# ZihanLiao/pytorch-kaldi-resnet

Measured on AMD Instinct MI355X. Metric: utterances/sec (300-frame x 80 fbank, bs256/GPU), ResNet-34 + AAM-softmax training step, higher is better.
Workload: dtype f32 (operands as 2 fp16 terms of value x 2^k, 3 cross products, f32 accumulate); 1 GPU; BASELINE configs[1]: ResNet-34 + AAM-softmax (m 0.2, s 30), 1211 speakers, 300-frame x 80 fbank, per-GPU batch 256, fwd+CE+bwd+SGD(0.9, wd 5e-4); global_batch=256, frames=300, feat_dim=80, parallelism=dp1, launch=hipGraph replay (1 graph), mfma=f16x3

## Files before the change

pytorch-kaldi-resnet_amd/csrc/conv3x3_c32_stream.hip:

```cpp
#include "spk_common.h"

struct Conv3x3C32Args {
    const float* in;
    const float* wpk;
    const unsigned* w_amax;
    float* out;
    const float* in_scale;
    const float* in_shift;
    float* stats;
    const unsigned* in_amax;
    unsigned* out_amax;
    int B, H, W, tiles_x, tiles_y, ntiles, flags;
};

#define C32_TH 8
#define C32_TW 16
#define C32_HW 18
#define C32_HP (10 * 18)
#define C32_PIX 144
#define C32_ROW 2816
#define C32_WBYTES (9 * 2 * 2 * 1024)
#ifndef C32_KD
#define C32_KD 2
#endif
#ifndef C32_DEPTH
#define C32_DEPTH 2
#endif

#ifdef C32_STAMPS
static __device__ unsigned long long g_c32_stamps[1024][8];
#define C32_T(i) do { const unsigned long long now_ = __builtin_amdgcn_s_memtime(); ph[i] += now_ - last; last = now_; } while (0)
#else
#define C32_T(i) do { } while (0)
#endif

#ifndef C32_XCD_BAND
#define C32_XCD_BAND 1
#endif
template <int VAR>
__global__ __launch_bounds__(256, 2) void conv3x3_c32_stream_kernel(Conv3x3C32Args a) {
    extern __shared__ __attribute__((aligned(16))) unsigned char lds3[];
    unsigned char* wl = lds3;
    unsigned char* hl = lds3 + C32_WBYTES;
    const int tid = threadIdx.x, lane = tid & 63;
    const int wave = __builtin_amdgcn_readfirstlane(tid >> 6);
    const int r = lane & 31, h = lane >> 5;
    constexpr bool AFF = VAR != 0;
    const float sig = spk_sigma_from_amax_bits(*a.in_amax);
    const float inv_sig = 1.f / sig, inv_wsig = 1.f / spk_sigma_from_amax_bits(*a.w_amax);
    const int H = a.H, W = a.W;

    for (int i = tid; i < C32_WBYTES / 16; i += 256) *(f32x4*)(wl + i * 16) = *(const f32x4*)(a.wpk + i * 4);

    const int q = tid & 7, prow = tid >> 3;
    int hy[6], hx[6];
    unsigned goff[6], loff[6];
#pragma unroll
    for (int u = 0; u < 6; ++u) {
        const int p = prow + 32 * u;
        const int pc = p < C32_HP ? p : C32_HP - 1;
        hy[u] = pc / C32_HW;
        hx[u] = pc - hy[u] * C32_HW;
        goff[u] = (unsigned)((hy[u] * W + hx[u]) * 32 + q * 4);
        loff[u] = (unsigned)(hy[u] * C32_ROW + hx[u] * C32_PIX + (q >> 2) * 64 + (q & 3) * 8);
    }
    const bool item5 = prow + 32 * 5 < C32_HP;
    f32x4 sc = {1.f, 1.f, 1.f, 1.f}, sh = {0.f, 0.f, 0.f, 0.f};
    if constexpr (AFF) {
        sc = *(const f32x4*)(a.in_scale + q * 4);
        sh = *(const f32x4*)(a.in_shift + q * 4);
    }

    f32x4 va[6], vb[6], vc[6];
    unsigned okma = 0, okmb = 0, okmc = 0;
    auto tile_origin = [&](int tile, int& b, int& y0, int& x0) {
        const int tx = tile % a.tiles_x;
        const int t2 = tile / a.tiles_x;
        const int ty = t2 % a.tiles_y;
        b = t2 / a.tiles_y;
        y0 = ty * C32_TH;
        x0 = tx * C32_TW;
    };
    auto issue = [&](int tile, f32x4* v, unsigned& okm) {
        int b, y0, x0;
        tile_origin(tile, b, y0, x0);
        const bool edge = y0 == 0 || y0 + C32_TH >= H || x0 == 0 || x0 + C32_TW >= W;
        const int base = ((b * H + y0 - 1) * W + x0 - 1) * 32;
        const int safe = ((b * H + y0) * W + x0) * 32 + q * 4;
        okm = 0x3f;
        if (!edge) {
#pragma unroll
            for (int u = 0; u < 6; ++u) v[u] = *(const f32x4*)(a.in + (unsigned)(base + (int)goff[u]));
        } else {
            okm = 0;
#pragma unroll
            for (int u = 0; u < 6; ++u) {
                const int iy = y0 - 1 + hy[u], ix = x0 - 1 + hx[u];
                const bool ok = iy >= 0 && iy < H && ix >= 0 && ix < W;
                okm |= (unsigned)ok << u;
                v[u] = *(const f32x4*)(a.in + (unsigned)(ok ? base + (int)goff[u] : safe));
            }
        }
    };

    double s_sum = 0.0, s_sq = 0.0;
    float out_mx = 0.f;
    const unsigned char* rd = hl + (2 * wave + (r >> 4)) * C32_ROW + (r & 15) * C32_PIX + h * 16;
    const unsigned char* wb = wl + lane * 16;

    const int G = (int)gridDim.x;
#ifdef C32_STAMPS
    unsigned long long ph[8] = {0, 0, 0, 0, 0, 0, 0, 0}, last = __builtin_amdgcn_s_memtime();
    const unsigned long long born = last;
#endif
    auto step = [&](int tile, f32x4* v, unsigned& okm) {
        int b, y0, x0;
        tile_origin(tile, b, y0, x0);
        C32_T(0);
        __syncthreads();
        C32_T(1);
#pragma unroll
        for (int u = 0; u < 6; ++u) {
#ifdef C32_ABL_NOSTAGE
            break;
#endif
            if (u == 5 && !item5) break;
            f32x4 w = v[u];
            if constexpr (AFF) {
                w = w * sc + sh;
                w[0] = fmaxf(w[0], 0.f);
                w[1] = fmaxf(w[1], 0.f);
                w[2] = fmaxf(w[2], 0.f);
                w[3] = fmaxf(w[3], 0.f);
            }
            if (!((okm >> u) & 1u)) w = (f32x4){0.f, 0.f, 0.f, 0.f};
            uint2 t0, t1;
            split2h(w, sig, t0, t1);
            *(uint2*)(hl + loff[u]) = t0;
            *(uint2*)(hl + loff[u] + 32) = t1;
        }
        C32_T(2);
        __syncthreads();
        C32_T(3);
#ifndef C32_ABL_NOLOAD
        if (tile + C32_DEPTH * G < a.ntiles) issue(tile + C32_DEPTH * G, v, okm);
#endif
        C32_T(4);

        f32x16 acc;
#pragma unroll
        for (int e = 0; e < 16; ++e) acc[e] = 0.f;
#ifdef C32_ABL_HALFK
        constexpr int NG = 1;
#else
        constexpr int NG = 2;
#endif
        constexpr int NS = NG * 9;
        f32x4 fr[C32_KD + 1][4];
        auto frag = [&](int s2, f32x4* f) {
            const int g = s2 / 9, t = s2 % 9;
            const int toff = (t / 3) * C32_ROW + (t % 3) * C32_PIX;
            f[0] = *(const f32x4*)(rd + toff + g * 64);
            f[1] = *(const f32x4*)(rd + toff + g * 64 + 32);
            f[2] = *(const f32x4*)(wb + ((t * 2 + g) * 2 + 0) * 1024);
            f[3] = *(const f32x4*)(wb + ((t * 2 + g) * 2 + 1) * 1024);
        };
#pragma unroll
        for (int s2 = 0; s2 < C32_KD; ++s2) frag(s2, fr[s2]);
#pragma unroll
        for (int s2 = 0; s2 < NS; ++s2) {
            if (s2 + C32_KD < NS) frag(s2 + C32_KD, fr[(s2 + C32_KD) % (C32_KD + 1)]);
            __builtin_amdgcn_sched_barrier(0);
            const f32x4* f = fr[s2 % (C32_KD + 1)];
            acc = __builtin_amdgcn_mfma_f32_32x32x16_f16(__builtin_bit_cast(f16x8, f[0]), __builtin_bit_cast(f16x8, f[3]), acc, 0, 0, 0);
            acc = __builtin_amdgcn_mfma_f32_32x32x16_f16(__builtin_bit_cast(f16x8, f[1]), __builtin_bit_cast(f16x8, f[2]), acc, 0, 0, 0);
            acc = __builtin_amdgcn_mfma_f32_32x32x16_f16(__builtin_bit_cast(f16x8, f[0]), __builtin_bit_cast(f16x8, f[2]), acc, 0, 0, 0);
            __builtin_amdgcn_sched_barrier(0);
        }

        C32_T(5);
        const bool ragged = y0 + C32_TH > H || x0 + C32_TW > W;
        float ts = 0.f, tq = 0.f, tile_mx = 0.f;
        float* ob = a.out + (size_t)((b * H + y0 + 2 * wave) * W + x0) * 32 + r;
#pragma unroll
        for (int e = 0; e < 16; ++e) {
            const int row = e >> 3, lx = (e & 3) + 8 * ((e >> 2) & 1) + 4 * h;
            if (ragged && (y0 + 2 * wave + row >= H || x0 + lx >= W)) continue;
            const float val = acc[e] * inv_sig * inv_wsig;
#ifndef C32_ABL_NOSTORE
            __builtin_nontemporal_store(val, ob + (row * W + lx) * 32);
#endif
            tile_mx = fmaxf(tile_mx, fabsf(val));
            ts += val;
            tq = __builtin_fmaf(val, val, tq);
        }
        if (__builtin_amdgcn_ballot_w64(!(tile_mx < __builtin_inff())) != 0) {
            tile_mx = 0.f;
#pragma unroll
            for (int e = 0; e < 16; ++e) {
                const int row = e >> 3, lx = (e & 3) + 8 * ((e >> 2) & 1) + 4 * h;
                if (ragged && (y0 + 2 * wave + row >= H || x0 + lx >= W)) continue;
                tile_mx = fmaxf(tile_mx, spk_finite_abs(acc[e] * inv_sig * inv_wsig));
            }
        }
        out_mx = fmaxf(out_mx, tile_mx);
        s_sum += (double)ts;
        s_sq += (double)tq;
        C32_T(6);
    };
    const int vblk = (C32_XCD_BAND && (G & 7) == 0) ? ((int)blockIdx.x & 7) * (G >> 3) + ((int)blockIdx.x >> 3) : (int)blockIdx.x;
    int tile = vblk;
    if (tile < a.ntiles) issue(tile, va, okma);
    if (tile + G < a.ntiles) issue(tile + G, vb, okmb);
    if (C32_DEPTH > 2 && tile + 2 * G < a.ntiles) issue(tile + 2 * G, vc, okmc);
    for (; tile < a.ntiles; tile += C32_DEPTH * G) {
        step(tile, va, okma);
        if (tile + G < a.ntiles) step(tile + G, vb, okmb);
        if (C32_DEPTH > 2 && tile + 2 * G < a.ntiles) step(tile + 2 * G, vc, okmc);
    }

#ifdef C32_STAMPS
    if (tid == 0 && blockIdx.x < 1024) {
        for (int i = 0; i < 7; ++i) g_c32_stamps[blockIdx.x][i] = ph[i];
        g_c32_stamps[blockIdx.x][7] = __builtin_amdgcn_s_memtime() - born;
    }
#endif
    if (a.out_amax) spk_wave_amax_commit(out_mx, a.out_amax);
    if (a.flags & SPK_EPI_STATS) {
        s_sum += __shfl_xor(s_sum, 32, 64);
        s_sq += __shfl_xor(s_sq, 32, 64);
        if (h == 0) {
            float* dst = a.stats + ((size_t)(vblk * 4 + wave) * 32 + r) * 2;
            dst[0] = (float)s_sum;
            dst[1] = (float)s_sq;
        }
    }
}

extern "C" int spk_conv3x3_c32_stream(const float* in, const float* wpk, float* out, const float* in_scale, const float* in_shift,
                                      float* stats , int B, int H, int W, int flags, const unsigned* in_amax,
                                      unsigned* out_amax, int nblocks, void* stream) {
    SPK_REQUIRE(in && wpk && out && in_amax, "spk_conv3x3_c32_stream: null pointer (in, wpk, out and the in_amax slot are required)");
    SPK_REQUIRE(B > 0 && H > 0 && W > 0 && (long long)B * H * W * 32 < 2147483647LL - 65536, "spk_conv3x3_c32_stream: %d x %d x %d pixels exceed 32-bit element offsets", B, H, W);
    SPK_REQUIRE((flags & ~(SPK_IN_AFFINE_RELU | SPK_EPI_STATS)) == 0, "spk_conv3x3_c32_stream: unsupported flags 0x%x", flags);
    SPK_REQUIRE(!(flags & SPK_IN_AFFINE_RELU) || (in_scale && in_shift), "spk_conv3x3_c32_stream: IN_AFFINE_RELU needs scale / shift");
    SPK_REQUIRE(!(flags & SPK_EPI_STATS) || stats, "spk_conv3x3_c32_stream: EPI_STATS needs a stats buffer");
    Conv3x3C32Args a;
    a.in = in; a.w_amax = (const unsigned*)wpk; a.wpk = wpk + 4; a.out = out; a.in_scale = in_scale; a.in_shift = in_shift;
    a.stats = stats; a.in_amax = in_amax; a.out_amax = out_amax; a.B = B; a.H = H; a.W = W; a.flags = flags;
    a.tiles_x = spk_ceil_div(W, C32_TW); a.tiles_y = spk_ceil_div(H, C32_TH);
    a.ntiles = B * a.tiles_y * a.tiles_x;
    SPK_REQUIRE(nblocks >= 1 && nblocks <= a.ntiles, "spk_conv3x3_c32_stream: nblocks=%d for %d tiles", nblocks, a.ntiles);
    const size_t lds_bytes = C32_WBYTES + 10 * C32_ROW;
    hipStream_t st = (hipStream_t)stream;
    if (flags & SPK_IN_AFFINE_RELU) hipLaunchKernelGGL(conv3x3_c32_stream_kernel<1>, dim3(nblocks), dim3(256), lds_bytes, st, a);
    else hipLaunchKernelGGL(conv3x3_c32_stream_kernel<0>, dim3(nblocks), dim3(256), lds_bytes, st, a);
    SPK_LAUNCH_CHECK("spk_conv3x3_c32_stream");
    return 0;
}

#ifdef C32_STAMPS
extern "C" int spk_debug_stamps_c32(unsigned long long* out, int nblocks) {
    if (nblocks < 0) {
        static unsigned long long zeros[1024][8];
        return (int)hipMemcpyToSymbol(HIP_SYMBOL(g_c32_stamps), zeros, sizeof(zeros));
    }
    return (int)hipMemcpyFromSymbol(out, HIP_SYMBOL(g_c32_stamps), sizeof(unsigned long long) * 8 * (size_t)nblocks);
}
#endif
```

Measured before the change: 5620 utt/s.

## Add optional 16x16x32 MFMA path and magic-number tile index division

Adds a compile-time C32_M16 variant of the 3x3 conv with 32 channels. It uses 16x16x32 f16 MFMAs over a 2x2 accumulator grid, with a new padded LDS layout for the halo and weights, per-lane stores of two output channels, and per-channel stats reduction. It also replaces the integer divide and modulo in tile_origin with multiply-high by precomputed reciprocals plus a correction step. The MFMA path is off by default (C32_M16=0), so only the cheaper tile index math runs by default.

New measurement: 5612 utt/s. About the same (-0.1%).

```diff
diff --git a/pytorch-kaldi-resnet_amd/csrc/conv3x3_c32_stream.hip b/pytorch-kaldi-resnet_amd/csrc/conv3x3_c32_stream.hip
--- a/pytorch-kaldi-resnet_amd/csrc/conv3x3_c32_stream.hip
+++ b/pytorch-kaldi-resnet_amd/csrc/conv3x3_c32_stream.hip
@@ -11,6 +11,7 @@
     const unsigned* in_amax;
     unsigned* out_amax;
     int B, H, W, tiles_x, tiles_y, ntiles, flags;
+    unsigned tiles_x_magic, tiles_y_magic;
 };
 
 #define C32_TH 8
@@ -20,8 +21,19 @@
 #define C32_PIX 144
 #define C32_ROW 2816
 #define C32_WBYTES (9 * 2 * 2 * 1024)
+#ifndef C32_M16
+#define C32_M16 0
+#endif
+#define C32M_PIX 160
+#define C32M_ROW (C32_HW * C32M_PIX)
+#define C32M_WROW 80
+#define C32M_WBYTES (9 * 2 * 32 * C32M_WROW)
 #ifndef C32_KD
+#if C32_M16
+#define C32_KD 1
+#else
 #define C32_KD 2
+#endif
 #endif
 #ifndef C32_DEPTH
 #define C32_DEPTH 2
@@ -40,17 +52,30 @@
 template <int VAR>
 __global__ __launch_bounds__(256, 2) void conv3x3_c32_stream_kernel(Conv3x3C32Args a) {
     extern __shared__ __attribute__((aligned(16))) unsigned char lds3[];
+#if C32_M16
+    unsigned char* wl = lds3;
+    unsigned char* hl = lds3 + C32M_WBYTES;
+#else
     unsigned char* wl = lds3;
     unsigned char* hl = lds3 + C32_WBYTES;
+#endif
     const int tid = threadIdx.x, lane = tid & 63;
     const int wave = __builtin_amdgcn_readfirstlane(tid >> 6);
     const int r = lane & 31, h = lane >> 5;
+    const int c16 = lane & 15, kq = lane >> 4;
     constexpr bool AFF = VAR != 0;
     const float sig = spk_sigma_from_amax_bits(*a.in_amax);
     const float inv_sig = 1.f / sig, inv_wsig = 1.f / spk_sigma_from_amax_bits(*a.w_amax);
     const int H = a.H, W = a.W;
 
+#if C32_M16
+    for (int i = tid; i < C32_WBYTES / 16; i += 256) {
+        const int wr = i & 31, wh = (i >> 5) & 1, wterm = (i >> 6) & 1, wg = (i >> 7) & 1, wt = i >> 8;
+        *(f32x4*)(wl + ((wt * 2 + wterm) * 32 + wr) * C32M_WROW + (2 * wg + wh) * 16) = *(const f32x4*)(a.wpk + i * 4);
+    }
+#else
     for (int i = tid; i < C32_WBYTES / 16; i += 256) *(f32x4*)(wl + i * 16) = *(const f32x4*)(a.wpk + i * 4);
+#endif
 
     const int q = tid & 7, prow = tid >> 3;
     int hy[6], hx[6];
@@ -62,8 +87,13 @@
         hy[u] = pc / C32_HW;
         hx[u] = pc - hy[u] * C32_HW;
         goff[u] = (unsigned)((hy[u] * W + hx[u]) * 32 + q * 4);
+#if C32_M16
+        loff[u] = (unsigned)(pc * C32M_PIX + q * 8);
+#else
         loff[u] = (unsigned)(hy[u] * C32_ROW + hx[u] * C32_PIX + (q >> 2) * 64 + (q & 3) * 8);
-    }
+#endif
+    }
+    constexpr int TERM1 = C32_M16 ? 64 : 32;
     const bool item5 = prow + 32 * 5 < C32_HP;
     f32x4 sc = {1.f, 1.f, 1.f, 1.f}, sh = {0.f, 0.f, 0.f, 0.f};
     if constexpr (AFF) {
@@ -74,12 +104,13 @@
     f32x4 va[6], vb[6], vc[6];
     unsigned okma = 0, okmb = 0, okmc = 0;
     auto tile_origin = [&](int tile, int& b, int& y0, int& x0) {
-        const int tx = tile % a.tiles_x;
-        const int t2 = tile / a.tiles_x;
-        const int ty = t2 % a.tiles_y;
-        b = t2 / a.tiles_y;
-        y0 = ty * C32_TH;
-        x0 = tx * C32_TW;
+        unsigned t2 = __umulhi((unsigned)tile, a.tiles_x_magic);
+        if ((unsigned)tile - t2 * (unsigned)a.tiles_x >= (unsigned)a.tiles_x) ++t2;
+        unsigned bb = __umulhi(t2, a.tiles_y_magic);
+        if (t2 - bb * (unsigned)a.tiles_y >= (unsigned)a.tiles_y) ++bb;
+        b = (int)bb;
+        y0 = (int)(t2 - bb * (unsigned)a.tiles_y) * C32_TH;
+        x0 = (int)((unsigned)tile - t2 * (unsigned)a.tiles_x) * C32_TW;
     };
     auto issue = [&](int tile, f32x4* v, unsigned& okm) {
         int b, y0, x0;
@@ -103,10 +134,16 @@
         }
     };
 
+    float out_mx = 0.f;
+#if C32_M16
+    double s_sum[2] = {0.0, 0.0}, s_sq[2] = {0.0, 0.0};
+    const unsigned char* rd = hl + (2 * wave * C32_HW + c16) * C32M_PIX + kq * 16;
+    const unsigned char* wb = wl + 2 * c16 * C32M_WROW + kq * 16;
+#else
     double s_sum = 0.0, s_sq = 0.0;
-    float out_mx = 0.f;
     const unsigned char* rd = hl + (2 * wave + (r >> 4)) * C32_ROW + (r & 15) * C32_PIX + h * 16;
     const unsigned char* wb = wl + lane * 16;
+#endif
 
     const int G = (int)gridDim.x;
 #ifdef C32_STAMPS
@@ -137,7 +174,7 @@
             uint2 t0, t1;
             split2h(w, sig, t0, t1);
             *(uint2*)(hl + loff[u]) = t0;
-            *(uint2*)(hl + loff[u] + 32) = t1;
+            *(uint2*)(hl + loff[u] + TERM1) = t1;
         }
         C32_T(2);
         __syncthreads();
@@ -147,6 +184,84 @@
 #endif
         C32_T(4);
 
+#if C32_M16
+        f32x4 acc[2][2];
+#pragma unroll
+        for (int i = 0; i < 4; ++i) acc[i >> 1][i & 1] = (f32x4){0.f, 0.f, 0.f, 0.f};
+#ifdef C32_ABL_HALFK
+        constexpr int NS = 5;
+#else
+        constexpr int NS = 9;
+#endif
+        f32x4 fr[C32_KD + 1][8];
+        auto frag = [&](int t, f32x4* f) {
+            const int toff = ((t / 3) * C32_HW + (t % 3)) * C32M_PIX;
+#pragma unroll
+            for (int i = 0; i < 2; ++i) {
+                f[2 * i] = *(const f32x4*)(rd + toff + i * C32M_ROW);
+                f[2 * i + 1] = *(const f32x4*)(rd + toff + i * C32M_ROW + 64);
+                f[4 + 2 * i] = *(const f32x4*)(wb + ((t * 2 + 0) * 32 + i) * C32M_WROW);
+                f[4 + 2 * i + 1] = *(const f32x4*)(wb + ((t * 2 + 1) * 32 + i) * C32M_WROW);
+            }
+        };
+#pragma unroll
+        for (int s2 = 0; s2 < C32_KD; ++s2) frag(s2, fr[s2]);
+#pragma unroll
+        for (int s2 = 0; s2 < NS; ++s2) {
+            if (s2 + C32_KD < NS) frag(s2 + C32_KD, fr[(s2 + C32_KD) % (C32_KD + 1)]);
+            __builtin_amdgcn_sched_barrier(0);
+            const f32x4* f = fr[s2 % (C32_KD + 1)];
+#pragma unroll
+            for (int pr = 0; pr < 3; ++pr) {
+                const int xt = pr == 1, wt = pr == 0;
+#pragma unroll
+                for (int i = 0; i < 2; ++i)
+#pragma unroll
+                    for (int j = 0; j < 2; ++j)
+                        acc[i][j] = __builtin_amdgcn_mfma_f32_16x16x32_f16(__builtin_bit_cast(f16x8, f[2 * i + xt]),
+                                                                           __builtin_bit_cast(f16x8, f[4 + 2 * j + wt]), acc[i][j], 0, 0, 0);
+            }
+            __builtin_amdgcn_sched_barrier(0);
+        }
+
+        C32_T(5);
+        typedef float f32x2 __attribute__((ext_vector_type(2)));
+        const bool ragged = y0 + C32_TH > H || x0 + C32_TW > W;
+        float ts[2] = {0.f, 0.f}, tq[2] = {0.f, 0.f}, tile_mx = 0.f;
+        float* ob = a.out + (size_t)((b * H + y0 + 2 * wave) * W + x0 + 4 * kq) * 32 + 2 * c16;
+#pragma unroll
+        for (int e = 0; e < 8; ++e) {
+            const int row = e >> 2, lx = 4 * kq + (e & 3);
+            if (ragged && (y0 + 2 * wave + row >= H || x0 + lx >= W)) continue;
+            f32x2 val;
+#pragma unroll
+            for (int j = 0; j < 2; ++j) {
+                val[j] = acc[row][j][e & 3] * inv_sig * inv_wsig;
+                tile_mx = fmaxf(tile_mx, fabsf(val[j]));
+                ts[j] += val[j];
+                tq[j] = __builtin_fmaf(val[j], val[j], tq[j]);
+            }
+#ifndef C32_ABL_NOSTORE
+            __builtin_nontemporal_store(val, (f32x2*)(ob + (row * W + (e & 3)) * 32));
+#endif
+        }
+        if (__builtin_amdgcn_ballot_w64(!(tile_mx < __builtin_inff())) != 0) {
+            tile_mx = 0.f;
+#pragma unroll
+            for (int e = 0; e < 8; ++e) {
+                const int row = e >> 2, lx = 4 * kq + (e & 3);
+                if (ragged && (y0 + 2 * wave + row >= H || x0 + lx >= W)) continue;
+#pragma unroll
+                for (int j = 0; j < 2; ++j) tile_mx = fmaxf(tile_mx, spk_finite_abs(acc[row][j][e & 3] * inv_sig * inv_wsig));
+            }
+        }
+        out_mx = fmaxf(out_mx, tile_mx);
+#pragma unroll
+        for (int j = 0; j < 2; ++j) {
+            s_sum[j] += (double)ts[j];
+            s_sq[j] += (double)tq[j];
+        }
+#else
         f32x16 acc;
 #pragma unroll
         for (int e = 0; e < 16; ++e) acc[e] = 0.f;
@@ -206,6 +321,7 @@
         out_mx = fmaxf(out_mx, tile_mx);
         s_sum += (double)ts;
         s_sq += (double)tq;
+#endif
         C32_T(6);
     };
     const int vblk = (C32_XCD_BAND && (G & 7) == 0) ? ((int)blockIdx.x & 7) * (G >> 3) + ((int)blockIdx.x >> 3) : (int)blockIdx.x;
@@ -227,6 +343,22 @@
 #endif
     if (a.out_amax) spk_wave_amax_commit(out_mx, a.out_amax);
     if (a.flags & SPK_EPI_STATS) {
+#if C32_M16
+#pragma unroll
+        for (int j = 0; j < 2; ++j) {
+            s_sum[j] += __shfl_xor(s_sum[j], 16, 64);
+            s_sq[j] += __shfl_xor(s_sq[j], 16, 64);
+            s_sum[j] += __shfl_xor(s_sum[j], 32, 64);
+            s_sq[j] += __shfl_xor(s_sq[j], 32, 64);
+        }
+        if (kq == 0) {
+            float* dst = a.stats + ((size_t)(vblk * 4 + wave) * 32 + 2 * c16) * 2;
+            dst[0] = (float)s_sum[0];
+            dst[1] = (float)s_sq[0];
+            dst[2] = (float)s_sum[1];
+            dst[3] = (float)s_sq[1];
+        }
+#else
         s_sum += __shfl_xor(s_sum, 32, 64);
         s_sq += __shfl_xor(s_sq, 32, 64);
         if (h == 0) {
@@ -234,6 +366,7 @@
             dst[0] = (float)s_sum;
             dst[1] = (float)s_sq;
         }
+#endif
     }
 }
 
@@ -251,7 +384,8 @@
     a.tiles_x = spk_ceil_div(W, C32_TW); a.tiles_y = spk_ceil_div(H, C32_TH);
     a.ntiles = B * a.tiles_y * a.tiles_x;
     SPK_REQUIRE(nblocks >= 1 && nblocks <= a.ntiles, "spk_conv3x3_c32_stream: nblocks=%d for %d tiles", nblocks, a.ntiles);
-    const size_t lds_bytes = C32_WBYTES + 10 * C32_ROW;
+    a.tiles_x_magic = 0xFFFFFFFFu / (unsigned)a.tiles_x; a.tiles_y_magic = 0xFFFFFFFFu / (unsigned)a.tiles_y;
+    const size_t lds_bytes = C32_M16 ? C32M_WBYTES + 10 * C32M_ROW : C32_WBYTES + 10 * C32_ROW;
     hipStream_t st = (hipStream_t)stream;
     if (flags & SPK_IN_AFFINE_RELU) hipLaunchKernelGGL(conv3x3_c32_stream_kernel<1>, dim3(nblocks), dim3(256), lds_bytes, st, a);
     else hipLaunchKernelGGL(conv3x3_c32_stream_kernel<0>, dim3(nblocks), dim3(256), lds_bytes, st, a);
```
